# TinyMPC/tinympc-matlab

Hardware: NVIDIA B200
Metric: solves_per_sec (higher is better)
Workload: dtype f32

## Files before the change

tinympc-matlab_b200/build.py:

```python
#!/usr/bin/env python3
from __future__ import annotations

import argparse
import os
import subprocess
import sys
from concurrent.futures import ThreadPoolExecutor
from pathlib import Path

HERE = Path(__file__).resolve().parent
CSRC = HERE / "csrc"
GEN = CSRC / "gen"
OBJ = HERE / "build"
LIB = HERE / "libtinympc_b200.so"
NVCC = os.environ.get("NVCC", "/usr/local/cuda/bin/nvcc")
ARCH = ["-gencode", "arch=compute_100a,code=sm_100a"]
FLAGS = ["-O3", "-std=c++17", "-lineinfo", "-Xcompiler", "-fPIC", "-Xptxas", "-v", "--expt-relaxed-constexpr"]

BOX, CON, ADP = 0, 1, 2
FEAT_NAME = {BOX: "box", CON: "con", ADP: "adp"}
FEAT_ENUM = {BOX: "FEAT_BOX", CON: "FEAT_CONSTR", ADP: "FEAT_ADAPT"}

REFS_NONE, REFS_SMEM, REFS_L2 = 0, 1, 2

# ... 7 lines not shown
    if tm:
        m = 1
    aff = ((nx, nu) == (6, 3)) if aff is None else aff
    opq = (bits == 64) if opq is None else opq
    return dict(aff=aff, tm=tm, ntm=ntm, opq=opq, tib=tib, bits=bits, nx=nx, nu=nu, N=N, feat=feat, refs=refs, ppb=ppb, variant=variant, block=block or b, minb=minb or m, fb=fb, gen=gen)


def plan_hybrid(nx, nu, N, max_warps=24):
    su = nu * (N - 1)
    for warps in range(max_warps, 3, -4):
        cols = 512 // (warps // 4)
        ttm = min(N - 1, cols // nx - (N - 2))
        if ttm < 0:
            continue
        smem_cols = 3 * su + (N - 1 - ttm) * nx
        if smem_cols * warps * 32 * 4 + 1024 + pack_elems(nx, nu, N) * 4 > 226 * 1024:
            continue
        if 65536 // (warps * 32) < 64 + 8 * nx:
            continue
        return warps, ttm
    return None


def inst3(nx, nu, N, refs=True, ppb=False, fb=False, variant=0, max_warps=24, opq=False, tib=None, aff=None, feat=BOX, cones=(0, 0, 0, 0, 0, 0), hyb=False, conv=-1):
    sx, su = nx * N, nu * (N - 1)
    ntm, nsm = (4, 5) if feat == CON else (2, 3)
    warps = min(max_warps, 4 * (512 // (ntm * sx)), ((226 * 1024 - 1024 - pack_elems(nx, nu, N) * 4) // (nsm * su * 4 * 32) // 4) * 4)
    ttm = -1
    if hyb:
        assert feat == BOX
        warps, ttm = plan_hybrid(nx, nu, N, max_warps)
    assert warps >= 4, "shape does not fit the incremental-form kernel"
    aff = ((nx, nu) == (6, 3)) if aff is None else aff
    tib = True if tib is None else tib
    return dict(gen=3, bits=32, nx=nx, nu=nu, N=N, feat=feat, refs=3 if refs else 0, ppb=ppb, fb=fb, variant=variant, block=warps * 32, aff=aff,
                opq=opq, tib=tib, tm=True, minb=1, ntm=ntm, cones=cones, ttm=ttm, conv=conv)


def inst4(nx, nu, N, refs=True, fb=False, variant=0, aff=None, cones=(0, 0, 0, 0, 0, 0)):
    scs, scd, ucs, ucd, nsl, nil = cones
    cw = 3 * nx + 2 * scd + 2 * nsl
    tm = (N - 1) * cw + 2 * nil * (N - 1)
    sm = 2 * (nu + ucd) * (N - 1) + nx * N + 2 * nu * (N - 1)
    warps = min(16, 4 * (512 // tm), ((226 * 1024 - 1024 - pack_elems(nx, nu, N) * 4) // (sm * 4 * 32) // 4) * 4)
    assert warps >= 4, "shape does not fit the mixed-precision kernel"
    aff = ((nx, nu) == (6, 3)) if aff is None else aff
    return dict(gen=4, bits=32, nx=nx, nu=nu, N=N, feat=CON, refs=3 if refs else 0, ppb=False, fb=fb, variant=variant, block=warps * 32, aff=aff,
                opq=False, tib=False, tm=True, minb=1, ntm=0, cones=cones, ttm=-1)


def instg(nx, nu, N, variant=0, adapt=False, cones=None, rolled=False, models=False):
    gs = 8 if nx + nu <= 8 else (16 if nx + nu <= 16 else 32)
    assert nx + nu <= 32
    assert not (models and (adapt or cones))
    return dict(gen=6 if models else 5, bits=64, nx=nx, nu=nu, N=N, feat=CON if cones else (ADP if adapt else BOX), refs=2, ppb=False, fb=False,
                variant=variant, block=128, aff=True, gs=gs, cones=cones, rolled=rolled)


def cols_per_thread(nx, nu, N, feat, refs, ntm=0):
# ... 16 lines not shown
        best = (0, 0)
        for ntm in range(1, (4 if feat == CON else 1) + 1):
            per_thread = cols_per_thread(nx, nu, N, feat, refs, ntm) * 4
            avail = budget_kb * 1024 - (1024 + pack_elems(nx, nu, N) * 4)
            warps = min(max_warps, avail // per_thread // 32, 4 * (512 // (ntm * nx * N)))
            warps = (warps // 4) * 4
            if warps > best[0]:
                best = (warps, ntm)
        return max(4, best[0]) * 32, max(1, best[1])
    per_thread = cols_per_thread(nx, nu, N, feat, refs) * bits // 8
    best = (32, 1, 0)
    for ctas in range(1, 9):
        avail = budget_kb * 1024 - ctas * (1024 + pack_elems(nx, nu, N) * bits // 8)
        block = min(256, (avail // ctas // per_thread // 32) * 32)
        while block >= 32 and (ctas * block // 32) % 4 != 0 and ctas * block > 128:
            block -= 32
        if block < 32:
            continue
        if ctas * block > best[2]:
            best = (block, ctas, ctas * block)
    return best[0], best[1]


def default_instances():
    out = []
    shapes = [(12, 4, 10), (4, 1, 20), (4, 1, 10), (6, 3, 10)]
    for (nx, nu, N) in shapes:
        hyb = plan_hybrid(nx, nu, N) is not None and plan_hybrid(nx, nu, N)[0] > inst3(nx, nu, N)["block"] // 32
        for fb in (True, False):
            out.append(inst3(nx, nu, N, refs=True, fb=fb, hyb=hyb))
            out.append(inst3(nx, nu, N, refs=False, fb=fb, hyb=hyb))
        out.append(inst3(nx, nu, N, refs=True, ppb=True, hyb=hyb))
    for fb in (True, False):
        out.append(inst4(6, 3, 10, refs=True, fb=fb, cones=(0, 3, 0, 3, 1, 1)))
        out.append(inst4(6, 3, 10, refs=True, fb=fb, cones=(0, 3, 0, 3, 0, 0)))
        out.append(inst3(6, 3, 10, refs=True, fb=fb, feat=CON, cones=(0, 3, 0, 3, 1, 1), variant=3))
        out.append(inst3(6, 3, 10, refs=True, fb=fb, feat=CON, cones=(0, 3, 0, 3, 0, 0), variant=3))
    for (nx, nu, N) in shapes:
        out.append(instg(nx, nu, N))
    out.append(instg(12, 4, 10, adapt=True))
    for (nx, nu, N) in shapes:
        out.append(instg(nx, nu, N, models=True))
    out.append(instg(6, 3, 10, cones=(0, 3, 0, 3, 1, 1)))
    out.append(instg(6, 3, 10, cones=(0, 3, 0, 3, 0, 0)))
    for bits in (32, 64):
        for (nx, nu, N) in shapes:
            if bits == 64:
                for fb in (True, False):
                    out.append(inst(bits, nx, nu, N, BOX, refs=REFS_L2, fb=fb, tm=True, variant=6))
                    out.append(inst(bits, nx, nu, N, BOX, refs=REFS_NONE, fb=fb, tm=True, variant=6))
                out.append(inst(bits, nx, nu, N, BOX, refs=REFS_L2, ppb=True, tm=True))
            out.append(inst(bits, nx, nu, N, CON, refs=REFS_L2, fb=True, tm=True, variant=0 if bits == 64 else 5))
            out.append(inst(bits, nx, nu, N, CON, refs=REFS_L2, tm=True, variant=0 if bits == 64 else 5))
            if (nx, nu) == (12, 4):
                out.append(inst(bits, nx, nu, N, ADP, refs=REFS_L2, fb=True, tm=True, variant=0 if bits == 32 else 6))
                out.append(inst(bits, nx, nu, N, ADP, refs=REFS_L2, tm=True, variant=0 if bits == 32 else 6))
    for (nx, nu, N) in shapes:
        if plan_hybrid(nx, nu, N) is not None and plan_hybrid(nx, nu, N)[0] > inst3(nx, nu, N)["block"] // 32:
            for fb in (True, False):
                out.append(inst3(nx, nu, N, refs=True, fb=fb, variant=9))
                out.append(inst3(nx, nu, N, refs=False, fb=fb, variant=9))
            out.append(inst3(nx, nu, N, refs=True, ppb=True, variant=9))
    out.append(inst3(12, 4, 10, refs=True, fb=True, hyb=True, variant=7, conv=0))
    out.append(inst(32, 12, 4, 10, BOX, refs=REFS_L2, variant=5, fb=True, tm=True))
    out.append(inst(32, 12, 4, 10, BOX, refs=REFS_L2, variant=5, tm=True))
    out.append(inst(32, 12, 4, 10, BOX, refs=REFS_L2, variant=5, ppb=True, tm=True))
    out.append(inst(32, 4, 1, 20, BOX, refs=REFS_NONE, variant=5, fb=True, tm=True))
    out.append(inst(32, 4, 1, 20, BOX, refs=REFS_L2, variant=5, fb=True, tm=True))
    return out


def name_of(i):
    t = "f32" if i["bits"] == 32 else "f64"
    if i["gen"] in (5, 6):
        cn = ("_c" + "".join(str(c) for c in i["cones"])) if i.get("cones") else ""
        return f"gpp_f64_{i['nx']}x{i['nu']}x{i['N']}_{FEAT_NAME[i['feat']]}{cn}_g{i['gs']}_v{i['variant']}{'_mdl' if i['gen'] == 6 else ''}"
    if i["gen"] == 4:
        cn = "_c" + "".join(str(c) for c in i["cones"])
        return f"tpp4_mix_{i['nx']}x{i['nu']}x{i['N']}_con{cn}{'' if i['refs'] else '_noref'}{'_fb' if i['fb'] else ''}{'_aff' if i['aff'] else ''}_v{i['variant']}"
    if i["gen"] == 3:
        cn = ("_c" + "".join(str(c) for c in i["cones"])) if i["feat"] == CON else ""
        return (f"tpp3_f32_{i['nx']}x{i['nu']}x{i['N']}_{FEAT_NAME[i['feat']]}{cn}{'' if i['refs'] else '_noref'}{'_ppb' if i['ppb'] else ''}{'_fb' if i['fb'] else ''}"
                f"{'_aff' if i['aff'] else ''}_v{i['variant']}")
    return (f"tpp{'' if i['gen'] == 1 else '2'}_{t}_{i['nx']}x{i['nu']}x{i['N']}_{FEAT_NAME[i['feat']]}{['_noref', '_refsm', ''][i['refs']]}"
            f"{'_ppb' if i['ppb'] else ''}{'_fb' if i['fb'] else ''}{'_aff' if (i['aff'] and i['gen'] == 2) else ''}{'_tm' if i['tm'] else ''}_v{i['variant']}")


def gen_sources(instances):
    GEN.mkdir(parents=True, exist_ok=True)
    names = []
    wanted = set()
    for i in instances:
        n = name_of(i)
        names.append(n)
        T = "float" if i["bits"] == 32 else "double"
        g = "" if i["gen"] == 1 else "2"
        b = lambda v: "true" if v else "false"
        if i["gen"] == 5:
            src = (
                "// generated by tinympc-matlab_b200/build.py -- do not edit\n"
                '#include "../tmpc_gpp.cuh"\n#include "../tmpc_registry.h"\nusing namespace tmpc;\n'
                f"using Cfg_{n} = GppCfg<{i['nx']}, {i['nu']}, {i['N']}, {i['gs']}, {i['block']}, {b(i['feat'] == ADP)}"
                + (f", {', '.join(str(c) for c in i['cones'])}, true" if i.get("cones") else (", 0, 0, 0, 0, 0, 0, false, true" if i.get("rolled") else "")) + ">;\n"
                f"TMPC_DEFINE_GPP_ENTRY({n}, Cfg_{n}, {i['variant']})\n"
            )
        elif i["gen"] == 6:
            src = (
                "// generated by tinympc-matlab_b200/build.py -- do not edit\n"
                '#include "../tmpc_gpp.cuh"\n#include "../tmpc_registry.h"\nusing namespace tmpc;\n'
                f"using Cfg_{n} = GppCfg<{i['nx']}, {i['nu']}, {i['N']}, {i['gs']}, {i['block']}, false, 0, 0, 0, 0, 0, 0, false, false>;\n"
                f"TMPC_DEFINE_GPP_MDL_ENTRY({n}, Cfg_{n}, {i['variant']})\n"
            )
        elif i["gen"] == 4:
            src = (
                "// generated by tinympc-matlab_b200/build.py -- do not edit\n"
                '#include "../tmpc_tpp4.cuh"\n#include "../tmpc_registry.h"\nusing namespace tmpc;\n'
                f"using Cfg_{n} = Tpp4Cfg<{i['nx']}, {i['nu']}, {i['N']}, {i['block']}, {b(i['refs'])}, {b(i['fb'])}, {b(i['aff'])}, "
                f"{', '.join(str(c) for c in i['cones'])}>;\n"
                f"TMPC_DEFINE_TPP4_ENTRY({n}, Cfg_{n}, {i['feat']}, 32, {i['variant']})\n"
            )
        elif i["gen"] == 3:
            src = (
                "// generated by tinympc-matlab_b200/build.py -- do not edit\n"
                '#include "../tmpc_tpp3.cuh"\n#include "../tmpc_registry.h"\nusing namespace tmpc;\n'
                f"using Cfg_{n} = Tpp3Cfg<{i['nx']}, {i['nu']}, {i['N']}, {i['block']}, {b(i['refs'])}, {b(i['ppb'])}, {b(i['fb'])}, {b(i['aff'])}, "
                f"{b(i['opq'])}, {b(i['tib'])}, {FEAT_ENUM[i['feat']]}, {', '.join(str(c) for c in i['cones'])}, {i['ttm']}, {i['conv']}>;\n"
                f"TMPC_DEFINE_TPP3_ENTRY({n}, Cfg_{n}, {i['feat']}, 32, {i['variant']})\n"
            )
        else:
          src = (
            "// generated by tinympc-matlab_b200/build.py -- do not edit\n"
            f'#include "../tmpc_tpp{g}.cuh"\n#include "../tmpc_registry.h"\nusing namespace tmpc;\n'
            f"using Cfg_{n} = Tpp{g}Cfg<{T}, {i['nx']}, {i['nu']}, {i['N']}, {FEAT_ENUM[i['feat']]}, {i['block']}, "
            f"{i['refs']}, {'true' if i['ppb'] else 'false'}, {i['minb']}, {'true' if i['fb'] else 'false'}"
            f"{((', true' if i['aff'] else ', false') + (', %d' % i['ntm']) + (', true' if i['opq'] else ', false') + (', true' if i['tib'] else ', false')) if g else ''}>;\n"
            f"TMPC_DEFINE_TPP{g}_ENTRY({n}, Cfg_{n}, {i['feat']}, {i['bits']}, {i['variant']})\n"
        )
        path = GEN / f"{n}.cu"
        wanted.add(path.name)
        if not path.exists() or path.read_text() != src:
            path.write_text(src)
    table = ["// generated by tinympc-matlab_b200/build.py -- do not edit", '#include "../tmpc_registry.h"', "namespace tmpc {"]
    table += [f"extern const KernelEntry {n};" for n in names]
    table.append("static const KernelEntry* const kTable[] = {" + ", ".join("&" + n for n in names) + "};")
    table.append("const KernelEntry* const* kernel_table(int* count) { *count = (int)(sizeof(kTable) / sizeof(kTable[0])); return kTable; }")
    table.append("}  // namespace tmpc\n")
    tpath = GEN / "tmpc_table.cu"
    wanted.add(tpath.name)
    txt = "\n".join(table)
# ... 72 lines not shown
```

tinympc-matlab_b200/csrc/tmpc_capi.cu:

```cuda
#include "../../include/tinympc_b200.h"

#include <cuda.h>
#include <cuda_runtime.h>

#include <algorithm>
#include <atomic>
#include <chrono>
#include <cmath>
#include <cstdio>
#include <cstdlib>
#include <cstring>
#include <limits>
#include <mutex>
#include <string>
#include <thread>
#include <vector>

#include "tmpc_common.h"
#include "tmpc_registry.h"
#include "tmpc_wpp.h"

using namespace tmpc;

namespace {

constexpr int kFeatBox = 0, kFeatConstr = 1, kFeatAdapt = 2;
constexpr int kMaxChunks = 64;
constexpr int kStreams = 3;
constexpr int kLatencyVariant = 9;
constexpr int kMaxStreamChunks = 256;

struct DevBuf {
    void* p = nullptr;
    size_t cap = 0;
    cudaError_t reserve(size_t bytes) {
        if (bytes <= cap) return cudaSuccess;
        if (p) cudaFree(p);
        p = nullptr; cap = 0;
        cudaError_t e = cudaMalloc(&p, bytes);
        if (e == cudaSuccess) cap = bytes;
        return e;
    }
// ... 14 lines not shown
    DevBuf x0, Xref, Uref, xmin, xmax, umin, umax, x, u, iter, status, res, rho, xrc, u0;
    DevBuf exp_xref[kStreams + 1], exp_x[kStreams + 1], exp_u[kStreams + 1];
    DevBuf ref_scratch[kStreams + 1];
    DevBuf wpp_scratch[kStreams + 1];
    DevBuf ref_scratch64[kStreams + 1];
    DevBuf marked[kStreams + 1];
    DevBuf order_buf;
    DevBuf models[14];
    cudaEvent_t ev_pass = nullptr, ev_copied = nullptr;
    int* qctl = nullptr;
    cudaStream_t fix_stream[kStreams + 1] = {nullptr, nullptr, nullptr, nullptr};
    cudaEvent_t ev_fork[kStreams + 1] = {nullptr, nullptr, nullptr, nullptr}, ev_join[kStreams + 1] = {nullptr, nullptr, nullptr, nullptr};
    cudaEvent_t ev_p0 = nullptr, ev_p1 = nullptr, ev_p2 = nullptr;
    bool pass_timed = false;
};

struct Family {
    bool set = false;
    int nx = 0, nu = 0, N = 0;
    int feat = kFeatBox;
    bool shared_bounds_ok = false;
    bool fastbox = false;
    bool affine = false;
    PackLayout L{};
    std::vector<double> pack;
    SolveParams base{};
};

}

struct tinympc_cuda_session;
struct tinympc_cuda_solver {
    std::vector<DeviceCtx> devs;
    Family fam;
    int precision = 32;
    int ctas_per_sm = 0;
    int chunks = 0;
    int variant = 0;
    int force_wpp = 0;
    int refill_min = 0;
    int streamed = 1;
    int compact_streamed = 1;
    int compact_early_d2h = 1;
    int order = 1;
    int order_sms = 1, order_from_div = 2;
    int compact_in_kernel = 1;
    double mixed_band = 0;
    int pass_timing = 0;
    int fixer_sms = -2;
    long long mixed_marked = 0;
    int mixed_pending_dev = -1;
    std::mutex mu;
    std::vector<tinympc_cuda_session*> sessions;
    std::string err;
    std::string last_kernel;
    std::atomic<long long> launches{0};
    double t_total_ms = 0, t_kernel_ms = 0;
    int t_chunks = 0;
};

struct tinympc_cuda_session {
    tinympc_cuda_solver* s = nullptr;
    int dev = 0, batch = 0, bits = 64;
// ... 18 lines not shown
}
int cuda_fail(tinympc_cuda_solver* s, cudaError_t e, const char* what) {
    return fail(s, TINYMPC_CUDA_ECUDA, std::string(what) + ": " + cudaGetErrorString(e));
}
struct DeviceGuard {
    int prev = 0;
    DeviceGuard() { cudaGetDevice(&prev); }
    ~DeviceGuard() { cudaSetDevice(prev); }
};
#define CU(s, call)                                              \
    do {                                                         \
        cudaError_t e__ = (call);                                \
        if (e__ != cudaSuccess) return cuda_fail(s, e__, #call); \
    } while (0)

void put_rowmajor(std::vector<double>& pk, int at, const double* src, int rows, int cols) {
    for (int r = 0; r < rows; ++r)
        for (int c = 0; c < cols; ++c) pk[at + r * cols + c] = src ? src[(size_t)c * rows + r] : 0.0;
}
void put_vec(std::vector<double>& pk, int at, const double* src, int n) {
    for (int i = 0; i < n; ++i) pk[at + i] = src ? src[i] : 0.0;
}

const KernelEntry* find_kernel(const Family& f, int bits, bool ppb, bool refs, int variant) {
    int n = 0;
    const KernelEntry* const* tab = kernel_table(&n);
    for (int pass = 0; pass < 2; ++pass) {
        for (int i = 0; i < n; ++i) {
            const KernelEntry* e = tab[i];
            if (e->models) continue;
            if (e->fastbox && (!f.fastbox || ppb)) continue;
            if (f.affine && !e->affine) continue;
            if (e->cone_fixed) {
                const SolveParams& b = f.base;
                const bool fsx = b.en_state_soc && b.n_state_cones > 0, fsu = b.en_input_soc && b.n_input_cones > 0;
                const bool okx = e->scd > 0 ? (fsx && b.n_state_cones == 1 && b.Acx[0] == e->scs && b.qcx[0] == e->scd) : !fsx;
                const bool oku = e->ucd > 0 ? (fsu && b.n_input_cones == 1 && b.Acu[0] == e->ucs && b.qcu[0] == e->ucd) : !fsu;
                if (!okx || !oku || f.L.nsl != e->nsl || f.L.nil != e->nil) continue;
                if ((e->nsl > 0 && !b.en_state_linear) || (e->nil > 0 && !b.en_input_linear)) continue;
            }
            if (e->family == KF_TPP && e->nx == f.nx && e->nu == f.nu && e->N == f.N && e->feat == f.feat && e->dtype_bits == bits &&
                e->ppb == (ppb ? 1 : 0) && e->variant == variant && ((e->refs != 0) == refs || (pass == 1 && e->refs != 0)))
                return e;
        }
    }
    if (variant != 0) return find_kernel(f, bits, ppb, refs, 0);
    return nullptr;
}

const KernelEntry* model_kernel(const tinympc_cuda_solver* s, const Family& f, bool ppb) {
    if (s->force_wpp || s->precision != 64 || f.feat != kFeatBox || ppb || !f.shared_bounds_ok || f.base.max_iter <= 0) return nullptr;
    int n = 0;
    const KernelEntry* const* tab = kernel_table(&n);
    for (int i = 0; i < n; ++i)
        if (tab[i]->models && tab[i]->nx == f.nx && tab[i]->nu == f.nu && tab[i]->N == f.N) return tab[i];
    return nullptr;
}

struct ModelField {
    const double* tinympc_cuda_models::*field;
    const char* name;
    int per_problem;
    bool required;
};
constexpr int kModelFields = 14;
void model_fields(int nx, int nu, bool adaptive, ModelField out[kModelFields]) {
    using M = tinympc_cuda_models;
    const ModelField f[kModelFields] = {
        {&M::Adyn, "Adyn", nx * nx, true}, {&M::Bdyn, "Bdyn", nx * nu, true}, {&M::fdyn, "fdyn", nx, false}, {&M::Q, "Q", nx, true},
// ... 139 lines not shown
    if (a.type != cudaMemoryTypeHost || a.devicePointer == nullptr) return false;
    *alias = a.devicePointer;
    return true;
}

int upload_family(tinympc_cuda_solver* s) {
    const Family& f = s->fam;
    std::vector<float> p32(f.pack.size());
    for (size_t i = 0; i < f.pack.size(); ++i) p32[i] = static_cast<float>(f.pack[i]);
    for (auto& d : s->devs) {
        CU(s, cudaSetDevice(d.device));
        if (d.pack32) cudaFree(d.pack32);
        if (d.pack64) cudaFree(d.pack64);
        d.pack32 = d.pack64 = nullptr;
        CU(s, cudaMalloc(&d.pack32, p32.size() * sizeof(float)));
        CU(s, cudaMalloc(&d.pack64, f.pack.size() * sizeof(double)));
        CU(s, cudaMemcpy(d.pack32, p32.data(), p32.size() * sizeof(float), cudaMemcpyHostToDevice));
        CU(s, cudaMemcpy(d.pack64, f.pack.data(), f.pack.size() * sizeof(double), cudaMemcpyHostToDevice));
    }
    return TINYMPC_CUDA_OK;
}

const KernelEntry* pick_kernel(const tinympc_cuda_solver* s, const DeviceCtx& d, const Family& f, int bits, bool ppb, bool refs, int batch) {
    const KernelEntry* ke = find_kernel(f, bits, ppb, refs, s->variant);
    if (ke && s->variant == 0 && bits == 32) {
        const KernelEntry* kl = find_kernel(f, bits, ppb, refs, kLatencyVariant);
        if (kl && kl->variant == kLatencyVariant && kl->block < ke->block && batch <= d.sm_count * kl->block) ke = kl;
    }
    return ke;
}

int launch_tpp(tinympc_cuda_solver* s, DeviceCtx& d, const KernelEntry* ke, SolveParams& p, DevBuf& rb, int bits, int* counter, cudaStream_t st,
               int reserve_sms = 0, int* grid_out = nullptr, int max_sms = 0, const tinympc_cuda_models* models = nullptr) {
    const Family& f = s->fam;
    const size_t smem = ke->smem_bytes(f.L.cold_size);
    if (smem > 227u * 1024u) return fail(s, TINYMPC_CUDA_EUNSUPPORTED, std::string("kernel ") + ke->name + " needs more shared memory than an SM has");
    CU(s, ke->prepare(smem));
    int occ = 0;
    CU(s, ke->occupancy(&occ, smem));
    if (occ < 1) return fail(s, TINYMPC_CUDA_EUNSUPPORTED, std::string("kernel ") + ke->name + " does not fit on an SM");
    if (s->ctas_per_sm > 0 && s->ctas_per_sm < occ) occ = s->ctas_per_sm;
    int grid = std::max(1, d.sm_count - reserve_sms) * occ;
    if (max_sms > 0) grid = std::min(grid, max_sms * occ);
    const int per_cta = ke->lanes_per_problem > 1 ? ke->block / ke->lanes_per_problem : ke->block;
    const int need = (p.batch + per_cta - 1) / per_cta;
    if (grid > need) grid = need;
    if (grid < 1) grid = 1;
    if (ke->refs == 2) {
        const size_t esz = bits == 64 ? sizeof(double) : sizeof(float);
// ... 859 lines not shown
            }
            for (int c = 0; c < nx; ++c) {
                double acc = 0;
                for (int r = 0; r < nx; ++r) acc += f.pack[L.AmBKt + c * nx + r] * p[r];
                pn[c] = acc + f.pack[L.APf + c];
            }
            p = pn;
        }
    }
    const double inf = std::numeric_limits<double>::infinity();
    const bool sb = fm->en_state_bound != 0, ib = fm->en_input_bound != 0;
    const bool have_sb = fm->x_min && fm->x_max, have_ib = fm->u_min && fm->u_max;
    for (int e = 0; e < nx * N; ++e) {
        f.pack[L.xmin + e] = (sb && have_sb) ? fm->x_min[e] : -inf;
        f.pack[L.xmax + e] = (sb && have_sb) ? fm->x_max[e] : inf;
    }
    for (int e = 0; e < nu * (N - 1); ++e) {
        f.pack[L.umin + e] = (ib && have_ib) ? fm->u_min[e] : -inf;
        f.pack[L.umax + e] = (ib && have_ib) ? fm->u_max[e] : inf;
    }
    f.shared_bounds_ok = (!sb || have_sb) && (!ib || have_ib);
    for (int r = 0; r < nx; ++r) f.affine = f.affine || f.pack[L.f + r] != 0.0 || f.pack[L.APf + r] != 0.0;
    for (int a = 0; a < nu; ++a) f.affine = f.affine || f.pack[L.BPf + a] != 0.0;
    f.fastbox = true;
    for (int e = 0; e < nx * N && f.fastbox; ++e)
        f.fastbox = f.pack[L.xmin + e] == f.pack[L.xmin + e % nx] && f.pack[L.xmax + e] == f.pack[L.xmax + e % nx] &&
                    f.pack[L.xmin + e] <= 0.0 && f.pack[L.xmax + e] >= 0.0;
    for (int e = 0; e < nu * (N - 1) && f.fastbox; ++e)
        f.fastbox = f.pack[L.umin + e] == f.pack[L.umin + e % nu] && f.pack[L.umax + e] == f.pack[L.umax + e % nu] &&
                    f.pack[L.umin + e] <= 0.0 && f.pack[L.umax + e] >= 0.0;
    for (int k = 0; k < nsl; ++k) {
        double nr = 0;
        for (int j = 0; j < nx; ++j) { double a = fm->Alin_x[(size_t)j * fm->numStateLinear + k]; f.pack[L.Alin_x + k * nx + j] = a; nr += a * a; }
        f.pack[L.blin_x + k] = fm->blin_x[k];
        f.pack[L.nrm_x + k] = nr;
    }
    for (int k = 0; k < nil; ++k) {
        double nr = 0;
        for (int j = 0; j < nu; ++j) { double a = fm->Alin_u[(size_t)j * fm->numInputLinear + k]; f.pack[L.Alin_u + k * nu + j] = a; nr += a * a; }
        f.pack[L.blin_u + k] = fm->blin_u[k];
        f.pack[L.nrm_u + k] = nr;
    }

    SolveParams& b = f.base;
    b = SolveParams{};
    b.rho = fm->rho;
// ... 415 lines not shown
        s->mixed_band = value;
    } else if (n == "pass_timing") {
        s->pass_timing = (int)value;
    } else if (n == "fixer_sms") {
        s->fixer_sms = (int)value;
    } else if (n == "force_wpp") {
        s->force_wpp = (int)value;
    } else if (n == "streamed") {
        s->streamed = value != 0;
    } else if (n == "compact_streamed") {
        s->compact_streamed = value != 0;
    } else if (n == "compact_early_d2h") {
        s->compact_early_d2h = value != 0;
    } else if (n == "order") {
        s->order = value != 0;
    } else if (n == "order_sms") {
        s->order_sms = (int)value;
    } else if (n == "order_from_div") {
        s->order_from_div = (int)value;
    } else if (n == "compact_in_kernel") {
        s->compact_in_kernel = value != 0;
    } else if (n == "refill_min") {
        s->refill_min = (int)value;
    } else {
        return fail(s, TINYMPC_CUDA_EINVAL, "unknown option " + n);
    }
    return TINYMPC_CUDA_OK;
}

int tinympc_cuda_num_devices(const tinympc_cuda_solver* s) { return s ? (int)s->devs.size() : 0; }
const char* tinympc_cuda_last_kernel(const tinympc_cuda_solver* s) { return s ? s->last_kernel.c_str() : ""; }
long long tinympc_cuda_launch_count(const tinympc_cuda_solver* s) { return s ? s->launches.load() : 0; }
int tinympc_cuda_last_timing(const tinympc_cuda_solver* s, double ms[3]) {
    if (!s || !ms) return TINYMPC_CUDA_EINVAL;
    ms[0] = s->t_total_ms; ms[1] = s->t_kernel_ms; ms[2] = (double)s->t_chunks;
    return TINYMPC_CUDA_OK;
}
int tinympc_cuda_last_pass_ms(tinympc_cuda_solver* s, double ms[2]) {
    if (!s || !ms) return TINYMPC_CUDA_EINVAL;
    ms[0] = ms[1] = 0.0;
    DeviceCtx& d = s->devs[0];
    if (!d.pass_timed) return TINYMPC_CUDA_ENOTREADY;
    int prev = 0;
    cudaGetDevice(&prev);
    cudaSetDevice(d.device);
    float a = 0.f, b = 0.f;
// ... 43 lines not shown
```

tinympc-matlab_b200/csrc/tmpc_registry.h:

```cpp
#pragma once
#include <cuda_runtime.h>

#include "tmpc_common.h"
#include "tmpc_wpp.h"

namespace tmpc {

enum KernelFamily : int { KF_TPP = 0, KF_WPP = 1 };

struct KernelEntry {
    const char* name;
    int family;
    int nx, nu, N;
    int feat;
    int dtype_bits;
    int refs;
    int ppb;
    int fastbox;
    int affine;
    int block;
    int variant;
    int streaming;
    size_t (*smem_bytes)(int pack_elems);
    cudaError_t (*prepare)(size_t smem);
    cudaError_t (*occupancy)(int* ctas_per_sm, size_t smem);
    cudaError_t (*launch)(const SolveParams& p, int grid, size_t smem, cudaStream_t st, const double* master_pack, const PackLayout& L);
    int cone_fixed;
    int scs, scd, ucs, ucd, nsl, nil;
    int lanes_per_problem;
    cudaError_t (*session_launch)(const SolveParams& p, int grid, size_t smem, cudaStream_t st, const double* master_pack, const PackLayout& L,
                                  double* ws, const WppLayout& W, int full);
    int compact_ok;
    int order_from_ok;
    int models;
    cudaError_t (*models_launch)(const SolveParams& p, int grid, size_t smem, cudaStream_t st, const double* master_pack, const PackLayout& L,
                                 const tinympc_cuda_models& m);
};

const KernelEntry* const* kernel_table(int* count);

}

#define TMPC_DEFINE_TPP2_ENTRY(SYM, CFG, FEATV, BITS, VAR)                                                          \
    namespace tmpc {                                                                                                \
    static size_t SYM##_smem(int pe) { return tpp2_smem_bytes<CFG>(pe); }                                           \
    static cudaError_t SYM##_prepare(size_t smem) {                                                                 \
        return cudaFuncSetAttribute(tpp2_kernel<CFG>, cudaFuncAttributeMaxDynamicSharedMemorySize, (int)smem);      \
    }                                                                                                               \
    static cudaError_t SYM##_occ(int* n, size_t smem) {                                                             \
        return cudaOccupancyMaxActiveBlocksPerMultiprocessor(n, tpp2_kernel<CFG>, CFG::BLOCK, smem);                \
    }                                                                                                               \
    static cudaError_t SYM##_launch(const SolveParams& p, int grid, size_t smem, cudaStream_t st, const double* mp, \
                                    const PackLayout& L) {                                                          \
        typename CFG::CPack cpk;                                                                                    \
        fill_const_pack2(cpk, mp, L);                                                                               \
        tpp2_kernel<CFG><<<grid, CFG::BLOCK, smem, st>>>(p, cpk);                                                   \
        return cudaGetLastError();                                                                                  \
    }                                                                                                               \
    extern const KernelEntry SYM = {#SYM, KF_TPP, CFG::NX, CFG::NU, CFG::NH, FEATV, BITS, CFG::REFMODE,             \
                                    CFG::PPB ? 1 : 0, CFG::FB ? 1 : 0, CFG::AFF ? 1 : 0, CFG::BLOCK, VAR, 1, SYM##_smem, SYM##_prepare, \
                                    SYM##_occ, SYM##_launch};                                 \
    }

#define TMPC_DEFINE_TPP3_ENTRY(SYM, CFG, FEATV, BITS, VAR)                                                          \
    namespace tmpc {                                                                                                \
    static size_t SYM##_smem(int pe) { return tpp3_smem_bytes<CFG>(pe); }                                           \
    static cudaError_t SYM##_prepare(size_t smem) {                                                                 \
        return cudaFuncSetAttribute(tpp3_kernel<CFG>, cudaFuncAttributeMaxDynamicSharedMemorySize, (int)smem);      \
    }                                                                                                               \
    static cudaError_t SYM##_occ(int* n, size_t smem) {                                                             \
        return cudaOccupancyMaxActiveBlocksPerMultiprocessor(n, tpp3_kernel<CFG>, CFG::BLOCK, smem);                \
    }                                                                                                               \
    static cudaError_t SYM##_launch(const SolveParams& p, int grid, size_t smem, cudaStream_t st, const double* mp, \
                                    const PackLayout& L) {                                                          \
        typename CFG::CPack cpk;                                                                                    \
        fill_const_pack3(cpk, mp, L);                                                                               \
        tpp3_kernel<CFG><<<grid, CFG::BLOCK, smem, st>>>(p, cpk);                                                   \
        return cudaGetLastError();                                                                                  \
    }                                                                                                               \
    extern const KernelEntry SYM = {#SYM, KF_TPP, CFG::NX, CFG::NU, CFG::NH, FEATV, BITS, CFG::REFMODE,             \
                                    CFG::PPB ? 1 : 0, CFG::FB ? 1 : 0, CFG::AFF ? 1 : 0, CFG::BLOCK, VAR, 1, SYM##_smem, SYM##_prepare, \
                                    SYM##_occ, SYM##_launch, CFG::CONSTR ? 1 : 0, CFG::SCS, CFG::SCD, CFG::UCS, CFG::UCD, CFG::NSL, CFG::NIL, \
                                    0, nullptr, 1, 1};                                                              \
    }

#define TMPC_DEFINE_TPP4_ENTRY(SYM, CFG, FEATV, BITS, VAR)                                                          \
    namespace tmpc {                                                                                                \
    static size_t SYM##_smem(int pe) { return tpp4_smem_bytes<CFG>(pe); }                                           \
    static cudaError_t SYM##_prepare(size_t smem) {                                                                 \
        return cudaFuncSetAttribute(tpp4_kernel<CFG>, cudaFuncAttributeMaxDynamicSharedMemorySize, (int)smem);      \
    }                                                                                                               \
    static cudaError_t SYM##_occ(int* n, size_t smem) {                                                             \
        return cudaOccupancyMaxActiveBlocksPerMultiprocessor(n, tpp4_kernel<CFG>, CFG::BLOCK, smem);                \
    }                                                                                                               \
    static cudaError_t SYM##_launch(const SolveParams& p, int grid, size_t smem, cudaStream_t st, const double* mp, \
                                    const PackLayout& L) {                                                          \
        typename CFG::CPack cpk;                                                                                    \
        fill_const_pack3(cpk, mp, L);                                                                               \
        tpp4_kernel<CFG><<<grid, CFG::BLOCK, smem, st>>>(p, cpk);                                                   \
        return cudaGetLastError();                                                                                  \
    }                                                                                                               \
    extern const KernelEntry SYM = {#SYM, KF_TPP, CFG::NX, CFG::NU, CFG::NH, FEATV, BITS, CFG::REFMODE,             \
                                    0, CFG::FB ? 1 : 0, CFG::AFF ? 1 : 0, CFG::BLOCK, VAR, 1, SYM##_smem, SYM##_prepare, \
                                    SYM##_occ, SYM##_launch, 1, CFG::SCS, CFG::SCD, CFG::UCS, CFG::UCD, CFG::NSL, CFG::NIL};                                 \
    }

// ... 59 lines not shown
```

tinympc-matlab_b200/csrc/tmpc_tpp2.cuh:

```cuda
#pragma once
#include <cuda_runtime.h>
#include <math_constants.h>

#include <cstring>
#include <type_traits>

#include "tmpc_common.h"

namespace tmpc {

enum : int { FEAT_BOX = 0, FEAT_CONSTR = 1, FEAT_ADAPT = 2 };
enum : int { REFS_NONE = 0, REFS_L2 = 2 };

__device__ __forceinline__ uint32_t smem_u32(const void* p) { return static_cast<uint32_t>(__cvta_generic_to_shared(p)); }
__device__ __forceinline__ void mbar_init(uint64_t* bar, uint32_t count) {
    asm volatile("mbarrier.init.shared::cta.b64 [%0], %1;" ::"r"(smem_u32(bar)), "r"(count) : "memory");
}
__device__ __forceinline__ void mbar_expect_tx(uint64_t* bar, uint32_t bytes) {
    asm volatile("mbarrier.arrive.expect_tx.shared::cta.b64 _, [%0], %1;" ::"r"(smem_u32(bar)), "r"(bytes) : "memory");
}
__device__ __forceinline__ void mbar_wait(uint64_t* bar, uint32_t parity) {
    uint32_t done = 0;
    do {
        asm volatile(
// ... 145 lines not shown
#pragma unroll
        for (int j = 0; j < NP; ++j) p[j] = mk2(v, v);
        t = v;
    }
};

#define TMPC_FOR_PAIRS(VecType, j) _Pragma("unroll") for (int j = 0; j < VecType::NP; ++j)

__host__ __device__ constexpr int pad2(int n) { return (n + 1) & ~1; }

template <int ROWS, int COLS, typename T>
__device__ __forceinline__ void mv_acc(const T* __restrict__ M0, int z, const Vec<T, COLS>& x, Vec<T, ROWS>& acc) {
    constexpr int RP = pad2(ROWS);
    const T* __restrict__ M = M0 + z;
#pragma unroll
    for (int c = 0; c < COLS; ++c) {
        const T xc = x.get(c);
#pragma unroll
        for (int j = 0; j < ROWS / 2; ++j) acc.p[j] = fmas(mk2(M[c * RP + 2 * j], M[c * RP + 2 * j + 1]), xc, acc.p[j]);
        if constexpr (ROWS & 1) acc.t = fmas(M[c * RP + ROWS - 1], xc, acc.t);
    }
}

template <typename T, int NX, int NU, int NH, bool ADAPT>
struct alignas(16) ConstPack2 {
    static constexpr int NXP = pad2(NX), NUP = pad2(NU);
    T A[NX * NXP];
    T B[NU * NXP];
    T NK[NX * NUP];
    T BT[NX * NUP];
    T Quu[NU * NUP];
    T AK[NX * NXP];
    T NKT[NU * NXP];
    T f[NXP], APf[NXP], BPf[NUP];
    T Qd[NXP], Rd[NUP];
    T xmin[NXP * NH], xmax[NXP * NH];
    T umin[NUP * (NH - 1)], umax[NUP * (NH - 1)];
    T NdK[ADAPT ? NX * NUP : 2], NdKT[ADAPT ? NU * NXP : 2], AT[ADAPT ? NX * NXP : 2];
};

template <typename T, int NX, int NU, int NH, bool ADAPT>
inline void fill_const_pack2(ConstPack2<T, NX, NU, NH, ADAPT>& c, const double* pk, const PackLayout& L) {
    constexpr int NXP = pad2(NX), NUP = pad2(NU);
    std::memset(&c, 0, sizeof(c));
    auto colmajor = [&](T* dst, int at, int rows, int cols, int RP, double sgn) {
        for (int r = 0; r < rows; ++r) for (int k = 0; k < cols; ++k) dst[k * RP + r] = static_cast<T>(sgn * pk[at + r * cols + k]);
// ... 1075 lines not shown
```

tinympc-matlab_b200/csrc/tmpc_tpp3.cuh:

```cuda
#pragma once
#include <type_traits>

#include "tmpc_tpp2.cuh"

#ifndef TMPC_TUNROLL_SMALL
#define TMPC_TUNROLL_SMALL 10
#endif

namespace tmpc {

enum : int { REFS_STATE = 3 };

template <int NX, int NU, int NH, int NSL, int NIL, bool CONV = false>
struct alignas(16) ConstPack3 : ConstPack2<float, NX, NU, NH, false> {
    float Alx[NSL > 0 ? NSL * NX : 1], blx[NSL > 0 ? NSL : 1], inx[NSL > 0 ? NSL : 1];
    float Alu[NIL > 0 ? NIL * NU : 1], blu[NIL > 0 ? NIL : 1], inu[NIL > 0 ? NIL : 1];
    float NG[CONV ? (NH - 1) * NX * pad2(NU) : 2], NQ[CONV ? NU * pad2(NU) : 2];
};
template <int NX, int NU, int NH, int NSL, int NIL, bool CONV>
inline void fill_const_pack3(ConstPack3<NX, NU, NH, NSL, NIL, CONV>& c, const double* pk, const PackLayout& L) {
    fill_const_pack2(static_cast<ConstPack2<float, NX, NU, NH, false>&>(c), pk, L);
    c.Alx[0] = c.blx[0] = c.inx[0] = c.Alu[0] = c.blu[0] = c.inu[0] = 0.f;
    c.NG[0] = c.NG[1] = c.NQ[0] = c.NQ[1] = 0.f;
    if constexpr (CONV) {
        constexpr int NUP = pad2(NU);
        double G[NU * NX], Gn[NU * NX];
        for (int a = 0; a < NU; ++a)
            for (int cc = 0; cc < NX; ++cc) {
                double acc = 0.0;
                for (int b = 0; b < NU; ++b) acc += pk[L.Quu_inv + a * NU + b] * pk[L.B + cc * NU + b];
                G[a * NX + cc] = acc;
            }
        for (int k = 0; k < NH - 1; ++k) {
            for (int a = 0; a < NU; ++a) for (int cc = 0; cc < NX; ++cc) c.NG[k * NX * NUP + cc * NUP + a] = static_cast<float>(-G[a * NX + cc]);
            for (int a = 0; a < NU; ++a)
                for (int cc = 0; cc < NX; ++cc) {
                    double acc = 0.0;
                    for (int r = 0; r < NX; ++r) acc += G[a * NX + r] * pk[L.AmBKt + r * NX + cc];
                    Gn[a * NX + cc] = acc;
                }
            for (int e = 0; e < NU * NX; ++e) G[e] = Gn[e];
        }
        for (int a = 0; a < NU; ++a) for (int b = 0; b < NU; ++b) c.NQ[b * NUP + a] = static_cast<float>(-pk[L.Quu_inv + a * NU + b]);
    }
    for (int k = 0; k < NSL; ++k) {
        for (int j = 0; j < NX; ++j) c.Alx[k * NX + j] = static_cast<float>(pk[L.Alin_x + k * NX + j]);
        c.blx[k] = static_cast<float>(pk[L.blin_x + k]);
        c.inx[k] = static_cast<float>(1.0 / pk[L.nrm_x + k]);
    }
    for (int k = 0; k < NIL; ++k) {
        for (int j = 0; j < NU; ++j) c.Alu[k * NU + j] = static_cast<float>(pk[L.Alin_u + k * NU + j]);
        c.blu[k] = static_cast<float>(pk[L.blin_u + k]);
        c.inu[k] = static_cast<float>(1.0 / pk[L.nrm_u + k]);
    }
}

template <int NX_, int NU_, int NH_, int BLOCK_, bool REFS_, bool PPB_, bool FB_, bool AFF_, bool OPQ_, bool TIB_, int FEAT_ = FEAT_BOX,
          int SCS_ = 0, int SCD_ = 0, int UCS_ = 0, int UCD_ = 0, int NSL_ = 0, int NIL_ = 0, int TTM_ = -1, int CONV_ = -1>
struct Tpp3Cfg {
    using T = float;
    static_assert(FEAT_ == FEAT_BOX || FEAT_ == FEAT_CONSTR, "the incremental form covers box and box + cone + half-space families");
    static constexpr int NX = NX_, NU = NU_, NH = NH_, FEAT = FEAT_, BLOCK = BLOCK_, MINB = 1;
    static constexpr bool CONSTR = FEAT_ == FEAT_CONSTR;
    static constexpr int SCS = SCS_, SCD = SCD_, UCS = UCS_, UCD = UCD_, NSL = NSL_, NIL = NIL_;
    static_assert(SCS_ >= 0 && SCS_ + SCD_ <= NX_ && UCS_ >= 0 && UCS_ + UCD_ <= NU_, "cone block outside the vector");
    static constexpr int REFMODE = REFS_ ? REFS_STATE : REFS_NONE;
    static constexpr bool REFS = REFS_;
    static constexpr bool PPB = PPB_;
    static constexpr bool FB = FB_ && !PPB_;
    static constexpr bool AFF = AFF_;
    static constexpr bool OPQ = OPQ_;
    static constexpr bool TIB = TIB_ && FB_ && !PPB_ && !OPQ_;
    static constexpr int SX = NX * NH, SU = NU * (NH - 1);
    static constexpr bool CONV = CONV_ < 0 ? (NX_ >= 12 && FEAT_ == FEAT_BOX) : (CONV_ != 0);
    using CPack = ConstPack3<NX_, NU_, NH_, NSL_, NIL_, CONV>;
    static constexpr bool HYB = TTM_ >= 0;
    static constexpr int TUNROLL = (NX_ <= 4 && FEAT_ == FEAT_BOX) ? TMPC_TUNROLL_SMALL : 1;
    static constexpr int TTM = HYB ? TTM_ : NH_;
    static_assert(!HYB || (FEAT_ == FEAT_BOX && NH_ >= 3 && TTM_ <= NH_ - 1), "hybrid layout: box instances only");
    static constexpr int oU = 0, oTZ = SU, oD = 2 * SU, oTZC = 3 * SU, oTZL = 4 * SU, oTS = 3 * SU;
    static constexpr int TS_STEPS = HYB ? (NH_ - 1 - TTM) : 0;
    static constexpr int COLS = (CONSTR ? 5 : 3) * SU + TS_STEPS * NX;
    static constexpr int TM_COLS_PER_THREAD = HYB ? ((NH_ - 2) + TTM) * NX : (CONSTR ? 4 : 2) * SX;
    static_assert(((BLOCK_ / 32 + 3) / 4) * TM_COLS_PER_THREAD <= 512, "the state does not fit the 512 tensor-memory columns");
};

__device__ __forceinline__ float2 sel0(bool c, float2 a) { return make_float2(c ? 0.f : a.x, c ? 0.f : a.y); }
__device__ __forceinline__ float sel0(bool c, float a) { return c ? 0.f : a; }

template <int S, int D, int N>
__device__ __forceinline__ void project_soc_fixed(Vec<float, N>& v, float mu, float inv_mu) {
    if constexpr (D > 0) {
        float ss = 0.f;
#pragma unroll
        for (int e = S; e < S + D - 1; ++e) ss = fmaf(v.get(e), v.get(e), ss);
        const float lv = v.get(S + D - 1);
        float a;
        asm("sqrt.approx.f32 %0, %1;" : "=f"(a) : "f"(ss));
// ... 357 lines not shown
                    if (!C::HYB || i + 1 <= NH - 2) X.issue(i + 1, xr);
                    VU du;
                    ND.load(i, du);
                    if constexpr (C::CONV) {
#pragma unroll
                        for (int j = 0; j < NU / 2; ++j) ND.setp(i, j, mk2(T(0), T(0)));
                        if constexpr (NU & 1) ND.sett(i, T(0));
                    }
                    if (i > 0 || anyff) mv_acc<NU, NX>(cp.NK, zf, dx, du);
                    VU un;
                    U.load(i, un);
#pragma unroll
                    for (int j = 0; j < NU / 2; ++j) un.p[j] = addv(un.p[j], du.p[j]);
                    if constexpr (NU & 1) un.t = un.t + du.t;
                    U.store(i, un);
                    VX dxn;
                    if constexpr (C::AFF) {
#pragma unroll
                        for (int j = 0; j < NX / 2; ++j) dxn.p[j] = ff ? mk2(cp.f[2 * j], cp.f[2 * j + 1]) : mk2(T(0), T(0));
                        if constexpr (NX & 1) dxn.t = ff ? cp.f[NX - 1] : T(0);
                    } else {
                        dxn.fill(T(0));
                    }
                    if (i > 0 || anyff) mv_acc<NX, NX>(cp.A, zf, dx, dxn);
                    mv_acc<NX, NU>(cp.B, zf, du, dxn);
                    dx = dxn;
                }
            }
            if constexpr (C::HYB) {
#pragma unroll
                for (int j = 0; j < NX / 2; ++j) xlast.p[j] = addv(xlast.p[j], dx.p[j]);
                if constexpr (NX & 1) xlast.t = xlast.t + dx.t;
            }
            X.stores_done();
        }
        publish_done(prm, unpub);
        k += 1;

        const bool first = (k == 1);
        const T nrho = -rho0;
        T rpx = 0, rdx = 0, rpu = 0, rdu = 0;
        auto slack = [&](auto traw, auto xv, auto lo, auto hi, T& rp, T& rd, auto& tnew, auto& dq) {
            const auto told = sel0(first, traw);
            const auto ref = subv(traw, told);
            auto vo = clampv(told, lo, hi);
            if constexpr (!C::FB) vo = sel0(first, vo);
            const auto go = subv(told, vo);
// ... 291 lines not shown
```

Before: 74.62 million.

## Specialize forward rollout A matvec to compile-time sparsity pattern of the dynamics

The build reads the A matrices of the quadrotor and cartpole problems and emits twin kernels whose A*dx product only issues FMAs for nonzero row pairs. The nonzeros are packed into a compact array in the constant pack. At runtime the kernel is selected only if the family's A pattern is covered by the compiled mask, otherwise the dense kernel is used, and a new dense_a option forces dense. This cuts FMAs and constant loads in the rollout, at the cost of more kernel instances and a build that depends on the problem definitions.

After: 80.00 million (median of 6 runs). 7.2% higher.

```diff
diff --git a/tinympc-matlab_b200/build.py b/tinympc-matlab_b200/build.py
--- a/tinympc-matlab_b200/build.py
+++ b/tinympc-matlab_b200/build.py
@@ -53,7 +53,7 @@
     return None
 
 
-def inst3(nx, nu, N, refs=True, ppb=False, fb=False, variant=0, max_warps=24, opq=False, tib=None, aff=None, feat=BOX, cones=(0, 0, 0, 0, 0, 0), hyb=False, conv=-1):
+def inst3(nx, nu, N, refs=True, ppb=False, fb=False, variant=0, max_warps=24, opq=False, tib=None, aff=None, feat=BOX, cones=(0, 0, 0, 0, 0, 0), hyb=False, conv=-1, sa=None):
     sx, su = nx * N, nu * (N - 1)
     ntm, nsm = (4, 5) if feat == CON else (2, 3)
     warps = min(max_warps, 4 * (512 // (ntm * sx)), ((226 * 1024 - 1024 - pack_elems(nx, nu, N) * 4) // (nsm * su * 4 * 32) // 4) * 4)
@@ -65,7 +65,7 @@
     aff = ((nx, nu) == (6, 3)) if aff is None else aff
     tib = True if tib is None else tib
     return dict(gen=3, bits=32, nx=nx, nu=nu, N=N, feat=feat, refs=3 if refs else 0, ppb=ppb, fb=fb, variant=variant, block=warps * 32, aff=aff,
-                opq=opq, tib=tib, tm=True, minb=1, ntm=ntm, cones=cones, ttm=ttm, conv=conv)
+                opq=opq, tib=tib, tm=True, minb=1, ntm=ntm, cones=cones, ttm=ttm, conv=conv, sa=sa)
 
 
 def inst4(nx, nu, N, refs=True, fb=False, variant=0, aff=None, cones=(0, 0, 0, 0, 0, 0)):
@@ -128,15 +128,42 @@
     return best[0], best[1]
 
 
+SPARSE_A_FAMILIES = {(12, 4, 10): "quadrotor", (4, 1, 20): "cartpole"}
+
+
+def load_problems():
+    import importlib.util
+    spec = importlib.util.spec_from_file_location("tmpc_build_problems", HERE / "problems.py")
+    mod = importlib.util.module_from_spec(spec)
+    sys.modules[spec.name] = mod
+    spec.loader.exec_module(mod)
+    return mod
+
+
+def a_pattern(A):
+    import numpy as np
+    A32 = np.asarray(A, dtype=np.float32)
+    nx = A32.shape[0]
+    return tuple(sum(1 << j for j in {r // 2 for r in range(nx) if A32[r, c] != 0}) for c in range(nx))
+
+
+def sparse_a_patterns():
+    P = load_problems()
+    return {shape: a_pattern(getattr(P, fam)().A) for shape, fam in SPARSE_A_FAMILIES.items()}
+
+
 def default_instances():
     out = []
     shapes = [(12, 4, 10), (4, 1, 20), (4, 1, 10), (6, 3, 10)]
+    sparse = sparse_a_patterns()
+    twins = lambda shape: (sparse[shape], None) if shape in sparse else (None,)
     for (nx, nu, N) in shapes:
         hyb = plan_hybrid(nx, nu, N) is not None and plan_hybrid(nx, nu, N)[0] > inst3(nx, nu, N)["block"] // 32
-        for fb in (True, False):
-            out.append(inst3(nx, nu, N, refs=True, fb=fb, hyb=hyb))
-            out.append(inst3(nx, nu, N, refs=False, fb=fb, hyb=hyb))
-        out.append(inst3(nx, nu, N, refs=True, ppb=True, hyb=hyb))
+        for sa in twins((nx, nu, N)):
+            for fb in (True, False):
+                out.append(inst3(nx, nu, N, refs=True, fb=fb, hyb=hyb, sa=sa))
+                out.append(inst3(nx, nu, N, refs=False, fb=fb, hyb=hyb, sa=sa))
+            out.append(inst3(nx, nu, N, refs=True, ppb=True, hyb=hyb, sa=sa))
     for fb in (True, False):
         out.append(inst4(6, 3, 10, refs=True, fb=fb, cones=(0, 3, 0, 3, 1, 1)))
         out.append(inst4(6, 3, 10, refs=True, fb=fb, cones=(0, 3, 0, 3, 0, 0)))
@@ -163,10 +190,11 @@
                 out.append(inst(bits, nx, nu, N, ADP, refs=REFS_L2, tm=True, variant=0 if bits == 32 else 6))
     for (nx, nu, N) in shapes:
         if plan_hybrid(nx, nu, N) is not None and plan_hybrid(nx, nu, N)[0] > inst3(nx, nu, N)["block"] // 32:
-            for fb in (True, False):
-                out.append(inst3(nx, nu, N, refs=True, fb=fb, variant=9))
-                out.append(inst3(nx, nu, N, refs=False, fb=fb, variant=9))
-            out.append(inst3(nx, nu, N, refs=True, ppb=True, variant=9))
+            for sa in twins((nx, nu, N)):
+                for fb in (True, False):
+                    out.append(inst3(nx, nu, N, refs=True, fb=fb, variant=9, sa=sa))
+                    out.append(inst3(nx, nu, N, refs=False, fb=fb, variant=9, sa=sa))
+                out.append(inst3(nx, nu, N, refs=True, ppb=True, variant=9, sa=sa))
     out.append(inst3(12, 4, 10, refs=True, fb=True, hyb=True, variant=7, conv=0))
     out.append(inst(32, 12, 4, 10, BOX, refs=REFS_L2, variant=5, fb=True, tm=True))
     out.append(inst(32, 12, 4, 10, BOX, refs=REFS_L2, variant=5, tm=True))
@@ -187,7 +215,7 @@
     if i["gen"] == 3:
         cn = ("_c" + "".join(str(c) for c in i["cones"])) if i["feat"] == CON else ""
         return (f"tpp3_f32_{i['nx']}x{i['nu']}x{i['N']}_{FEAT_NAME[i['feat']]}{cn}{'' if i['refs'] else '_noref'}{'_ppb' if i['ppb'] else ''}{'_fb' if i['fb'] else ''}"
-                f"{'_aff' if i['aff'] else ''}_v{i['variant']}")
+                f"{'_aff' if i['aff'] else ''}{'_sa' if i.get('sa') else ''}_v{i['variant']}")
     return (f"tpp{'' if i['gen'] == 1 else '2'}_{t}_{i['nx']}x{i['nu']}x{i['N']}_{FEAT_NAME[i['feat']]}{['_noref', '_refsm', ''][i['refs']]}"
             f"{'_ppb' if i['ppb'] else ''}{'_fb' if i['fb'] else ''}{'_aff' if (i['aff'] and i['gen'] == 2) else ''}{'_tm' if i['tm'] else ''}_v{i['variant']}")
 
@@ -230,7 +258,8 @@
                 "// generated by tinympc-matlab_b200/build.py -- do not edit\n"
                 '#include "../tmpc_tpp3.cuh"\n#include "../tmpc_registry.h"\nusing namespace tmpc;\n'
                 f"using Cfg_{n} = Tpp3Cfg<{i['nx']}, {i['nu']}, {i['N']}, {i['block']}, {b(i['refs'])}, {b(i['ppb'])}, {b(i['fb'])}, {b(i['aff'])}, "
-                f"{b(i['opq'])}, {b(i['tib'])}, {FEAT_ENUM[i['feat']]}, {', '.join(str(c) for c in i['cones'])}, {i['ttm']}, {i['conv']}>;\n"
+                f"{b(i['opq'])}, {b(i['tib'])}, {FEAT_ENUM[i['feat']]}, {', '.join(str(c) for c in i['cones'])}, {i['ttm']}, {i['conv']}"
+                + (f", SparsePairs<{', '.join(f'{m}u' for m in i['sa'])}>" if i.get("sa") else "") + ">;\n"
                 f"TMPC_DEFINE_TPP3_ENTRY({n}, Cfg_{n}, {i['feat']}, 32, {i['variant']})\n"
             )
         else:
diff --git a/tinympc-matlab_b200/csrc/tmpc_capi.cu b/tinympc-matlab_b200/csrc/tmpc_capi.cu
--- a/tinympc-matlab_b200/csrc/tmpc_capi.cu
+++ b/tinympc-matlab_b200/csrc/tmpc_capi.cu
@@ -18,6 +18,7 @@
 
 #include "tmpc_common.h"
 #include "tmpc_registry.h"
+#include "tmpc_sparse_a.h"
 #include "tmpc_wpp.h"
 
 using namespace tmpc;
@@ -78,6 +79,7 @@
     bool shared_bounds_ok = false;
     bool fastbox = false;
     bool affine = false;
+    std::vector<unsigned> a_pairs;
     PackLayout L{};
     std::vector<double> pack;
     SolveParams base{};
@@ -95,6 +97,7 @@
     int variant = 0;
     int force_wpp = 0;
     int refill_min = 0;
+    int dense_a = 0;
     int streamed = 1;
     int compact_streamed = 1;
     int compact_early_d2h = 1;
@@ -159,7 +162,7 @@
     for (int i = 0; i < n; ++i) pk[at + i] = src ? src[i] : 0.0;
 }
 
-const KernelEntry* find_kernel(const Family& f, int bits, bool ppb, bool refs, int variant) {
+const KernelEntry* find_kernel(const Family& f, int bits, bool ppb, bool refs, int variant, bool dense_a = false) {
     int n = 0;
     const KernelEntry* const* tab = kernel_table(&n);
     for (int pass = 0; pass < 2; ++pass) {
@@ -168,6 +171,8 @@
             if (e->models) continue;
             if (e->fastbox && (!f.fastbox || ppb)) continue;
             if (f.affine && !e->affine) continue;
+            if (e->a_cols && (dense_a || !a_pattern_covers(e->a_pairs, e->a_cols, f.a_pairs.data(), (int)f.a_pairs.size())))
+                continue;
             if (e->cone_fixed) {
                 const SolveParams& b = f.base;
                 const bool fsx = b.en_state_soc && b.n_state_cones > 0, fsu = b.en_input_soc && b.n_input_cones > 0;
@@ -181,7 +186,7 @@
                 return e;
         }
     }
-    if (variant != 0) return find_kernel(f, bits, ppb, refs, 0);
+    if (variant != 0) return find_kernel(f, bits, ppb, refs, 0, dense_a);
     return nullptr;
 }
 
@@ -367,9 +372,9 @@
 }
 
 const KernelEntry* pick_kernel(const tinympc_cuda_solver* s, const DeviceCtx& d, const Family& f, int bits, bool ppb, bool refs, int batch) {
-    const KernelEntry* ke = find_kernel(f, bits, ppb, refs, s->variant);
+    const KernelEntry* ke = find_kernel(f, bits, ppb, refs, s->variant, s->dense_a);
     if (ke && s->variant == 0 && bits == 32) {
-        const KernelEntry* kl = find_kernel(f, bits, ppb, refs, kLatencyVariant);
+        const KernelEntry* kl = find_kernel(f, bits, ppb, refs, kLatencyVariant, s->dense_a);
         if (kl && kl->variant == kLatencyVariant && kl->block < ke->block && batch <= d.sm_count * kl->block) ke = kl;
     }
     return ke;
@@ -1275,6 +1280,8 @@
     f.shared_bounds_ok = (!sb || have_sb) && (!ib || have_ib);
     for (int r = 0; r < nx; ++r) f.affine = f.affine || f.pack[L.f + r] != 0.0 || f.pack[L.APf + r] != 0.0;
     for (int a = 0; a < nu; ++a) f.affine = f.affine || f.pack[L.BPf + a] != 0.0;
+    f.a_pairs.assign(nx, 0u);
+    a_pairs_of(f.pack.data() + L.A, nx, f.a_pairs.data());
     f.fastbox = true;
     for (int e = 0; e < nx * N && f.fastbox; ++e)
         f.fastbox = f.pack[L.xmin + e] == f.pack[L.xmin + e % nx] && f.pack[L.xmax + e] == f.pack[L.xmax + e % nx] &&
@@ -1736,6 +1743,8 @@
         s->compact_in_kernel = value != 0;
     } else if (n == "refill_min") {
         s->refill_min = (int)value;
+    } else if (n == "dense_a") {
+        s->dense_a = value != 0;
     } else {
         return fail(s, TINYMPC_CUDA_EINVAL, "unknown option " + n);
     }
diff --git a/tinympc-matlab_b200/csrc/tmpc_registry.h b/tinympc-matlab_b200/csrc/tmpc_registry.h
--- a/tinympc-matlab_b200/csrc/tmpc_registry.h
+++ b/tinympc-matlab_b200/csrc/tmpc_registry.h
@@ -35,6 +35,8 @@
     int models;
     cudaError_t (*models_launch)(const SolveParams& p, int grid, size_t smem, cudaStream_t st, const double* master_pack, const PackLayout& L,
                                  const tinympc_cuda_models& m);
+    int a_cols;
+    const unsigned* a_pairs;
 };
 
 const KernelEntry* const* kernel_table(int* count);
@@ -81,7 +83,7 @@
     extern const KernelEntry SYM = {#SYM, KF_TPP, CFG::NX, CFG::NU, CFG::NH, FEATV, BITS, CFG::REFMODE,             \
                                     CFG::PPB ? 1 : 0, CFG::FB ? 1 : 0, CFG::AFF ? 1 : 0, CFG::BLOCK, VAR, 1, SYM##_smem, SYM##_prepare, \
                                     SYM##_occ, SYM##_launch, CFG::CONSTR ? 1 : 0, CFG::SCS, CFG::SCD, CFG::UCS, CFG::UCD, CFG::NSL, CFG::NIL, \
-                                    0, nullptr, 1, 1};                                                              \
+                                    0, nullptr, 1, 1, 0, nullptr, CFG::SA::NCOL, CFG::SA::kCols};                  \
     }
 
 #define TMPC_DEFINE_TPP4_ENTRY(SYM, CFG, FEATV, BITS, VAR)                                                          \
diff --git a/tinympc-matlab_b200/csrc/tmpc_sparse_a.h b/tinympc-matlab_b200/csrc/tmpc_sparse_a.h
--- /dev/null
+++ b/tinympc-matlab_b200/csrc/tmpc_sparse_a.h
@@ -0,0 +1,20 @@
+#pragma once
+
+namespace tmpc {
+
+inline void a_pairs_of(const double* A_rowmajor, int nx, unsigned* cols) {
+    for (int c = 0; c < nx; ++c) cols[c] = 0u;
+    for (int r = 0; r < nx; ++r)
+        for (int c = 0; c < nx; ++c)
+            if (static_cast<float>(A_rowmajor[r * nx + c]) != 0.f) cols[c] |= 1u << (r / 2);
+}
+
+inline bool a_pattern_covers(const unsigned* inst, int inst_cols, const unsigned* fam, int nx) {
+    if (inst_cols == 0) return true;
+    if (inst_cols != nx) return false;
+    for (int c = 0; c < nx; ++c)
+        if (fam[c] & ~inst[c]) return false;
+    return true;
+}
+
+}
diff --git a/tinympc-matlab_b200/csrc/tmpc_tpp2.cuh b/tinympc-matlab_b200/csrc/tmpc_tpp2.cuh
--- a/tinympc-matlab_b200/csrc/tmpc_tpp2.cuh
+++ b/tinympc-matlab_b200/csrc/tmpc_tpp2.cuh
@@ -191,6 +191,60 @@
     }
 }
 
+template <unsigned... M>
+struct SparsePairs {
+    static constexpr int NCOL = static_cast<int>(sizeof...(M));
+    static constexpr bool DENSE = NCOL == 0;
+    static constexpr unsigned kCols[NCOL + 1] = {M..., 0u};
+    __host__ __device__ static constexpr unsigned col(int c) {
+        unsigned r = 0;
+        int i = 0;
+        ((r |= (i++ == c ? M : 0u)), ...);
+        return r;
+    }
+    __host__ __device__ static constexpr int pairs(int rows) {
+        int n = 0;
+        for (int c = 0; c < NCOL; ++c)
+            for (int j = 0; j < rows / 2; ++j) n += (col(c) >> j) & 1u;
+        return n;
+    }
+    __host__ __device__ static constexpr int packed(int rows) {
+        int n = 2 * pairs(rows);
+        if (rows & 1)
+            for (int c = 0; c < NCOL; ++c) n += (col(c) >> (rows / 2)) & 1u;
+        return n;
+    }
+    template <typename T>
+    static void pack(T* dst, const T* M0, int rows) {
+        const int rp = pad2(rows);
+        int k = 0;
+        for (int c = 0; c < NCOL; ++c)
+            for (int j = 0; j < rows / 2; ++j)
+                if ((col(c) >> j) & 1u) { dst[k++] = M0[c * rp + 2 * j]; dst[k++] = M0[c * rp + 2 * j + 1]; }
+        if (rows & 1)
+            for (int c = 0; c < NCOL; ++c)
+                if ((col(c) >> (rows / 2)) & 1u) dst[k++] = M0[c * rp + rows - 1];
+    }
+};
+
+template <class S, int ROWS, int COLS, typename T>
+__device__ __forceinline__ void mv_acc_masked(const T* __restrict__ MP, int z, const Vec<T, COLS>& x, Vec<T, ROWS>& acc) {
+    static_assert(S::NCOL == COLS, "pattern of another shape");
+    constexpr int NPAIR = S::pairs(ROWS);
+    const T* __restrict__ M = MP + z;
+    int k = 0, kt = 2 * NPAIR;
+#pragma unroll
+    for (int c = 0; c < COLS; ++c) {
+        const T xc = x.get(c);
+#pragma unroll
+        for (int j = 0; j < ROWS / 2; ++j)
+            if ((S::col(c) >> j) & 1u) { acc.p[j] = fmas(mk2(M[2 * k], M[2 * k + 1]), xc, acc.p[j]); ++k; }
+        if constexpr (ROWS & 1) {
+            if ((S::col(c) >> (ROWS / 2)) & 1u) { acc.t = fmas(M[kt], xc, acc.t); ++kt; }
+        }
+    }
+}
+
 template <typename T, int NX, int NU, int NH, bool ADAPT>
 struct alignas(16) ConstPack2 {
     static constexpr int NXP = pad2(NX), NUP = pad2(NU);
diff --git a/tinympc-matlab_b200/csrc/tmpc_tpp3.cuh b/tinympc-matlab_b200/csrc/tmpc_tpp3.cuh
--- a/tinympc-matlab_b200/csrc/tmpc_tpp3.cuh
+++ b/tinympc-matlab_b200/csrc/tmpc_tpp3.cuh
@@ -11,17 +11,20 @@
 
 enum : int { REFS_STATE = 3 };
 
-template <int NX, int NU, int NH, int NSL, int NIL, bool CONV = false>
+template <int NX, int NU, int NH, int NSL, int NIL, bool CONV = false, class SA = SparsePairs<>>
 struct alignas(16) ConstPack3 : ConstPack2<float, NX, NU, NH, false> {
     float Alx[NSL > 0 ? NSL * NX : 1], blx[NSL > 0 ? NSL : 1], inx[NSL > 0 ? NSL : 1];
     float Alu[NIL > 0 ? NIL * NU : 1], blu[NIL > 0 ? NIL : 1], inu[NIL > 0 ? NIL : 1];
     float NG[CONV ? (NH - 1) * NX * pad2(NU) : 2], NQ[CONV ? NU * pad2(NU) : 2];
+    float AS[SA::packed(NX) > 2 ? SA::packed(NX) : 2];
 };
-template <int NX, int NU, int NH, int NSL, int NIL, bool CONV>
-inline void fill_const_pack3(ConstPack3<NX, NU, NH, NSL, NIL, CONV>& c, const double* pk, const PackLayout& L) {
+template <int NX, int NU, int NH, int NSL, int NIL, bool CONV, class SA>
+inline void fill_const_pack3(ConstPack3<NX, NU, NH, NSL, NIL, CONV, SA>& c, const double* pk, const PackLayout& L) {
     fill_const_pack2(static_cast<ConstPack2<float, NX, NU, NH, false>&>(c), pk, L);
     c.Alx[0] = c.blx[0] = c.inx[0] = c.Alu[0] = c.blu[0] = c.inu[0] = 0.f;
     c.NG[0] = c.NG[1] = c.NQ[0] = c.NQ[1] = 0.f;
+    c.AS[0] = c.AS[1] = 0.f;
+    if constexpr (!SA::DENSE) SA::pack(c.AS, c.A, NX);
     if constexpr (CONV) {
         constexpr int NUP = pad2(NU);
         double G[NU * NX], Gn[NU * NX];
@@ -56,7 +59,8 @@
 }
 
 template <int NX_, int NU_, int NH_, int BLOCK_, bool REFS_, bool PPB_, bool FB_, bool AFF_, bool OPQ_, bool TIB_, int FEAT_ = FEAT_BOX,
-          int SCS_ = 0, int SCD_ = 0, int UCS_ = 0, int UCD_ = 0, int NSL_ = 0, int NIL_ = 0, int TTM_ = -1, int CONV_ = -1>
+          int SCS_ = 0, int SCD_ = 0, int UCS_ = 0, int UCD_ = 0, int NSL_ = 0, int NIL_ = 0, int TTM_ = -1, int CONV_ = -1,
+          class SA_ = SparsePairs<>>
 struct Tpp3Cfg {
     using T = float;
     static_assert(FEAT_ == FEAT_BOX || FEAT_ == FEAT_CONSTR, "the incremental form covers box and box + cone + half-space families");
@@ -73,7 +77,9 @@
     static constexpr bool TIB = TIB_ && FB_ && !PPB_ && !OPQ_;
     static constexpr int SX = NX * NH, SU = NU * (NH - 1);
     static constexpr bool CONV = CONV_ < 0 ? (NX_ >= 12 && FEAT_ == FEAT_BOX) : (CONV_ != 0);
-    using CPack = ConstPack3<NX_, NU_, NH_, NSL_, NIL_, CONV>;
+    using SA = SA_;
+    static_assert(SA_::DENSE || SA_::NCOL == NX_, "A pattern of another shape");
+    using CPack = ConstPack3<NX_, NU_, NH_, NSL_, NIL_, CONV, SA_>;
     static constexpr bool HYB = TTM_ >= 0;
     static constexpr int TUNROLL = (NX_ <= 4 && FEAT_ == FEAT_BOX) ? TMPC_TUNROLL_SMALL : 1;
     static constexpr int TTM = HYB ? TTM_ : NH_;
@@ -477,7 +483,10 @@
                     } else {
                         dxn.fill(T(0));
                     }
-                    if (i > 0 || anyff) mv_acc<NX, NX>(cp.A, zf, dx, dxn);
+                    if (i > 0 || anyff) {
+                        if constexpr (C::SA::DENSE) mv_acc<NX, NX>(cp.A, zf, dx, dxn);
+                        else mv_acc_masked<typename C::SA, NX, NX>(cp.AS, zf, dx, dxn);
+                    }
                     mv_acc<NX, NU>(cp.B, zf, du, dxn);
                     dx = dxn;
                 }
```
